# ska-sa/katsdpsigproc

Measured on AMD Instinct MI355X. Metric: visibility samples/s (baselines x channels) through full RFI flagger, higher is better.
Workload: dtype f32 amplitude / f64 deviations

## Files before the change

katsdpsigproc_amd/csrc/fused_common.h:

```cpp
#pragma once
#include <stdlib.h>

#include "bitplane.h"
#include "median_merge.h"
#include "median_window.h"

#ifndef FUSED_MAD_BITS
#define FUSED_MAD_BITS 1
#endif
#ifndef FUSED_STRIP
#define FUSED_STRIP 4
#endif
#define FUSED_THREADS (64 * FUSED_STRIP)
#define FUSED_MAD_NORMAL 1.4826

#ifdef KSP_DIAG_REALTIME
#define FUSED_DIAG_CLOCK() __builtin_amdgcn_s_memrealtime()
#else
#define FUSED_DIAG_CLOCK() __builtin_amdgcn_s_memtime()
#endif
#ifdef KSP_DIAG
#define FUSED_DIAG_STOP(p) ((p).debug_stop)
#define FUSED_DIAG_TRACE(p) ((p).trace)
#else
// ... 621 lines not shown
#pragma unroll
            for (int bit = 6; bit >= 0; bit--) step1(bit);
        } else {
#pragma unroll
            for (int bit = 14; bit >= 0; bit--) step1(bit);
        }
        if (top_hint != nullptr) *top_hint = (int)(K >> 7);
#else
#pragma unroll
        for (int bit = 14; bit >= 2; bit -= 2) step2(bit, bit - 1);
        step1(0);
#endif
        in_bin = ksp_wave_sum_dpp(__popc(eq0) + __popc(eq1));
    } else {
        zeros_keys = zeros;
        if (ksp_any(tiny != 0)) zeros -= ksp_wave_sum(tiny);
        if (zeros == total) return __builtin_nan("");
        rank2 = total + zeros;
        rank = rank2 / 2;
        if (rank < zeros_keys) return 0x1p-150 * FUSED_MAD_NORMAL;
        for (int bit = 14; bit >= 0; bit--) {
            const unsigned test = K | (1u << bit);
            const int c = count_less16<NP>(kp, test);
            if (c <= rank) {
                K = test;
                below_bin = c;
            }
        }
        in_bin = count_less16<NP>(kp, K + 1) - below_bin;
    }
    const bool even = !(rank2 & 1);
    stamp(10);
    if (debug_stop == 32) return (double)(K + below_bin);
    auto key_of = [&](int j) -> unsigned {
        return min((__float_as_uint(dv(j)) & 0x7fffffffu) + 0xffffu, 0x7fffffffu) >> 16;
    };
    auto bin_mask = [&](unsigned key) -> unsigned long long {
        unsigned long long m = 0;
#pragma unroll
        for (int j = 0; j < R; j++)
            if (key_of(j) == key) m |= 1ull << j;
        return m;
    };
    int r = rank - below_bin;
    unsigned long long cand = 0;
    const bool narrowed = in_bin > LIST_CAP;
    if (narrowed) {
        const unsigned first = ((K - 1) << 16) + 1u;
        unsigned offs = 0;
        int below = below_bin;
        for (int bit = 15; bit >= 0; bit--) {
            const unsigned test = first + (offs | (1u << bit));
            int c = 0;
#pragma unroll
            for (int j = 0; j < R; j++) c += (__float_as_uint(dv(j)) & 0x7fffffffu) < test;
            c = ksp_wave_sum(c);
            if (c <= rank) {
                offs |= 1u << bit;
                below = c;
            }
        }
        const unsigned cur = first + offs;
        cand = 0;
#pragma unroll
        for (int j = 0; j < R; j++)
            if ((__float_as_uint(dv(j)) & 0x7fffffffu) == cur) cand |= 1ull << j;
        in_bin = ksp_wave_sum(__popcll(cand));
        r = rank - below;
        below_bin = below;
        if (in_bin > LIST_CAP) {
            auto each = [&](auto &&f) {
                unsigned long long todo = cand;
                while (__any(todo != 0)) {
                    const bool has = todo != 0;
                    const int j = has ? __ffsll((long long)todo) - 1 : 0;
                    todo &= todo - 1;
                    const double x = fabs(exact_dev<WIDTH>(c0 + j, fetch));
                    if (has) f(x);
                }
            };
            double lo = __builtin_inf(), hi = 0.0;
            each([&](double x) {
                lo = fmin(lo, x);
                hi = fmax(hi, x);
            });
            lo = ksp_wave_min(lo);
            hi = ksp_wave_max(hi);
            double xk = lo, prev = lo;
            if (lo != hi) {
                const unsigned long long base = (unsigned long long)__double_as_longlong(lo);
                const unsigned long long span = (unsigned long long)__double_as_longlong(hi) - base;
                unsigned long long offs = 0;
                int below_k = 0;
                for (int bit = 63 - __clzll((long long)span); bit >= 0; bit--) {
                    const unsigned long long test = base + (offs | (1ull << bit));
                    int c = 0;
                    each([&](double x) {
                        c += (unsigned long long)__double_as_longlong(x) < test;
                    });
                    c = ksp_wave_sum(c);
                    if (c <= r) {
                        offs |= 1ull << bit;
                        below_k = c;
                    }
                }
                xk = __longlong_as_double((long long)(base + offs));
                prev = xk;
                if (even && r >= 1 && below_k == r) {
                    double m = 0.0;
                    each([&](double x) { m = (x < xk) ? fmax(m, x) : m; });
                    prev = ksp_wave_max(m);
                }
            }
            if (even && r == 0) {
                float b32 = 0.0f;
#pragma unroll
                for (int j = 0; j < R; j++) {
                    const float a = fabsf(dv(j));
                    b32 = (__float_as_uint(a) < cur) ? fmaxf(b32, a) : b32;
                }
                b32 = ksp_wave_max(b32);
                unsigned long long bm = 0;
#pragma unroll
                for (int j = 0; j < R; j++)
                    if (fabsf(dv(j)) == b32) bm |= 1ull << j;
                const int n2 = gather_exact<WIDTH>(bm, c0, list, 0, LIST_CAP, fetch);
                double below_max = 0.0;
                for (int i = lane; i < min(n2, LIST_CAP); i += 64) below_max = fmax(below_max, list[i]);
                below_max = ksp_wave_max(below_max);
                __builtin_amdgcn_wave_barrier();
                if (n2 > LIST_CAP) {
                    unsigned long long todo = bm;
                    double m = 0.0;
                    while (__any(todo != 0)) {
                        const bool has = todo != 0;
                        const int j = has ? __ffsll((long long)todo) - 1 : 0;
                        todo &= todo - 1;
                        const double x = fabs(exact_dev<WIDTH>(c0 + j, fetch));
                        m = has ? fmax(m, x) : m;
                    }
                    below_max = ksp_wave_max(m);
                }
                prev = below_max;
            }
            if (even) xk = (xk + prev) / 2.0;
            return xk * FUSED_MAD_NORMAL;
        }
    }
    double xk, prev;
    bool have_prev;
    if (!narrowed && in_bin <= 64) {
        int *lc = (int *)list;
        int n = 0;
        auto place = [&](bool hit, int channel) {
            const unsigned long long m = ksp_ballot(hit);
            const int pos = n + __builtin_amdgcn_mbcnt_hi((unsigned)(m >> 32),
                                                         __builtin_amdgcn_mbcnt_lo((unsigned)m, 0));
            if (hit) lc[pos] = channel;
            n += __popcll(m);
        };
        double x;
        bool ranked = false;
        unsigned *lv = (unsigned *)lc + 128;
        static_assert(LIST_CAP * 2 >= 128 + 64 + 8, "candidate values behind the channel numbers");
        if constexpr (R == 64 && HAVE_EXACT) {
            const int mine = __popc(eq0) + __popc(eq1);
            const int incl = ksp_wave_scan_dpp(mine);
            n = __builtin_amdgcn_readlane(incl, 63);
            int pos = incl - mine;
            unsigned h0 = eq0, h1 = eq1;
            while (ksp_any((h0 | h1) != 0)) {
                const bool has = (h0 | h1) != 0;
                int j = 0;
                if (h0) {
                    j = 2 * (__ffs((int)h0) - 1);
                    h0 &= h0 - 1;
                } else if (h1) {
                    j = 2 * (__ffs((int)h1) - 1) + 1;
                    h1 &= h1 - 1;
                }
                const float v = ksp_select_dev<R>(dev, j);
                if (has) {
                    lc[pos] = (c0 + j) | (((exact >> j) & 1) ? (int)0x80000000 : 0);
                    lv[pos] = __float_as_uint(v) & 0x7fffffffu;
                    pos++;
                }
            }
            if (lane < 8) lv[n + lane] = 0xffffffffu;
            __builtin_amdgcn_fence(__ATOMIC_RELEASE, "wavefront");
            __builtin_amdgcn_wave_barrier();
            const int slot = lane < n ? lane : 0;
            const int e0 = lc[slot];
            const unsigned a32 = lv[slot];
            x = (double)__uint_as_float(a32);
            const bool inexact = lane < n && e0 >= 0;
            stamp(11);
            if (debug_stop == 33) return x;
            if (ksp_any(inexact)) {
                const double xe = fabs(exact_dev<WIDTH>(e0 & 0x7fffffff, fetch));
                x = inexact ? xe : x;
            } else {
                unsigned k32, p32;
                rank_list_u32(lv, a32, n, r, lane, k32, p32, have_prev);
                xk = (double)__uint_as_float(k32);
                prev = (double)__uint_as_float(p32);
                ranked = true;
            }
        } else {
            if constexpr (R == 64) {
                const int mine = __popc(eq0) + __popc(eq1);
                const int incl = ksp_wave_scan_dpp(mine);
                n = __builtin_amdgcn_readlane(incl, 63);
                int pos = incl - mine;
                unsigned h0 = eq0, h1 = eq1;
                while (h0 | h1) {
                    if (h0) {
                        lc[pos++] = c0 + 2 * (__ffs((int)h0) - 1);
                        h0 &= h0 - 1;
                    } else {
                        lc[pos++] = c0 + 2 * (__ffs((int)h1) - 1) + 1;
                        h1 &= h1 - 1;
                    }
                }
            } else {
#pragma unroll
                for (int j = 0; j < R; j++) place(key_of(j) == K, c0 + j);
            }
            __builtin_amdgcn_fence(__ATOMIC_RELEASE, "wavefront");
            __builtin_amdgcn_wave_barrier();
            const int c = lc[lane < n ? lane : 0];
            stamp(11);
            if (debug_stop == 33) return (double)c;
            x = fabs(exact_dev<WIDTH>(c, fetch));
        }
        stamp(12);
        if (!ranked) rank_lanes64(x, n, r, lane, xk, prev, have_prev);
        stamp(13);
        __builtin_amdgcn_wave_barrier();
    } else {
        gather_exact<WIDTH>(narrowed ? cand : bin_mask(K), c0, list, 0, LIST_CAP, fetch);
        rank_in_list(list, in_bin, r, lane, xk, prev, have_prev);
        __builtin_amdgcn_wave_barrier();
    }
    if (even && !have_prev) {
        int k2 = -1;
#pragma unroll
        for (int j = 0; j < R; j++) {
            const int kj = (int)key_of(j);
            k2 = (kj < (int)K) ? max(k2, kj) : k2;
        }
        k2 = wave_max_int(k2);
        const bool below_is_tiny = k2 <= 0;
        unsigned long long bm = bin_mask((unsigned)(below_is_tiny ? 0 : k2));
        float b32 = 0.0f;
#pragma unroll
        for (int j = 0; j < R; j++)
            if ((bm >> j) & 1) b32 = fmaxf(b32, fabsf(dv(j)));
        b32 = ksp_wave_max(b32);
        unsigned long long top = 0;
#pragma unroll
        for (int j = 0; j < R; j++)
            if (((bm >> j) & 1) && fabsf(dv(j)) == b32) top |= 1ull << j;
        bool recompute = true;
        if (below_is_tiny) {
            prev = 0x1p-150;
            recompute = false;
        }
        if constexpr (HAVE_EXACT) {
            if (recompute && !ksp_any((top & ~exact) != 0)) {
                prev = (double)b32;
                recompute = false;
            }
        }
        if (recompute) {
            const int n2 = gather_exact<WIDTH>(top, c0, list, 0, LIST_CAP, fetch);
            double below_max = 0.0;
            for (int i = lane; i < min(n2, LIST_CAP); i += 64) below_max = fmax(below_max, list[i]);
            prev = ksp_wave_max(below_max);
            __builtin_amdgcn_wave_barrier();
            if (n2 > LIST_CAP) {
                double m = 0.0;
                while (__any(top != 0)) {
                    const bool has = top != 0;
                    const int j = has ? __ffsll((long long)top) - 1 : 0;
                    top &= top - 1;
                    const double x = fabs(exact_dev<WIDTH>(c0 + j, fetch));
                    m = has ? fmax(m, x) : m;
                }
                prev = ksp_wave_max(m);
            }
        }
    }
    stamp(14);
    if (even) xk = (xk + prev) / 2.0;
    return xk * FUSED_MAD_NORMAL;
}

template <int WIDTH, class Fetch>
__device__ __noinline__ double exact_dev_call(int c, Fetch fetch)
{
    return exact_dev<WIDTH>(c, fetch);
}

template <int WIDTH, class Fetch>
__device__ __forceinline__ unsigned long long threshold_wide(const FusedParams &p,
                                                             const float (&dev)[64],
                                                             unsigned long long fl,
                                                             unsigned long long ge, double t1,
                                                             bool positive, int lane, int C,
                                                             Fetch &&fetch)
{
    const int c0 = lane * 64;
    float nmax = 0.0f;
#pragma unroll
    for (int j = 0; j < 64; j++) nmax = fmaxf(nmax, -dev[j]);
    nmax = ksp_wave_max(nmax);
    float U[64];
    unsigned Nb[16];
#pragma unroll
    for (int j = 0; j < 64; j++) U[j] = dev[j];
#pragma unroll
    for (int q = 0; q < 16; q++) Nb[q] = 0;
    int lvl = -1;
    float umax = 0.0f;
    bool counted = false;
    auto level = [&](auto s_) {
        constexpr int s = decltype(s_)::value;
        ksp_static_for<s>([&](auto r_) {
            constexpr int r = decltype(r_)::value;
            const float e = __shfl_down(U[r], 1, 64);
#pragma unroll
            for (int j = r; j + s < 64; j += s) U[j] += U[j + s];
            U[r + 64 - s] += e;
        });
        if (counted) {
            if constexpr (s >= 4) {
                constexpr int sq = s / 4;
                ksp_static_for<sq>([&](auto r_) {
                    constexpr int r = decltype(r_)::value;
                    const unsigned e = (unsigned)__shfl_down((int)Nb[r], 1, 64);
#pragma unroll
                    for (int q = r; q + sq < 16; q += sq) Nb[q] += Nb[q + sq];
                    Nb[r + 16 - sq] += e;
                });
            } else {
                const unsigned e = (unsigned)__shfl_down((int)Nb[0], 1, 64);
#pragma unroll
                for (int q = 0; q < 16; q++)
                    Nb[q] += __builtin_amdgcn_alignbyte(q + 1 < 16 ? Nb[(q + 1) % 16] : e, Nb[q], s);
            }
        }
    };
#pragma unroll 1
    for (int k = 0; k < p.n_windows; k++) {
        if (positive && !ksp_any((ge & ~fl) != 0)) break;
        const int w = 1 << k;
        const double scale = k == 0 ? p.scales[0] : k == 1 ? p.scales[1] : k == 2 ? p.scales[2]
                           : k == 3 ? p.scales[3] : k == 4 ? p.scales[4] : k == 5 ? p.scales[5]
                           : k == 6 ? p.scales[6] : p.scales[7];
        const float thrf = (float)(t1 * scale);
        const float limf = __fmul_rn(thrf, (float)w);
        const double limit = (double)limf;
        if (positive && lvl >= 0 && umax < thrf) continue;
        if (lvl < 0) {
            counted = ksp_any(fl != 0);
            {
                const unsigned f_lo = (unsigned)fl, f_hi = (unsigned)(fl >> 32);
#pragma unroll
                for (int j = 0; j < 64; j++)
                    U[j] = (((j < 32 ? f_lo : f_hi) >> (j & 31)) & 1u) ? 0.0f : dev[j];
            }
            float m = U[0];
#pragma unroll
            for (int j = 1; j < 64; j++) m = fmaxf(m, U[j]);
            umax = ksp_wave_max(m);
            if (counted) {
#pragma unroll
                for (int q = 0; q < 16; q++)
                    Nb[q] = ((((unsigned)(fl >> (4 * q))) & 0xfu) * 0x00204081u) & 0x01010101u;
            }
            lvl = 0;
            if (positive && umax < thrf) continue;
        }
        while (lvl < k) {
            switch (lvl) {
            case 0: level(std::integral_constant<int, 1>{}); break;
            case 1: level(std::integral_constant<int, 2>{}); break;
            case 2: level(std::integral_constant<int, 4>{}); break;
            case 3: level(std::integral_constant<int, 8>{}); break;
            case 4: level(std::integral_constant<int, 16>{}); break;
            case 5: level(std::integral_constant<int, 32>{}); break;
            default: level(std::integral_constant<int, 64>{}); break;
            }
            lvl++;
        }
        const int nvalid = C - w + 1 - c0;
        const unsigned long long valid = nvalid >= 64 ? ~0ull : nvalid <= 0 ? 0ull : ((1ull << nvalid) - 1);
        unsigned long long hits = 0, unsure = valid;
        if (positive) {
            unsigned h_lo = 0, h_hi = 0, m_lo = 0, m_hi = 0;
            const float c = (float)w * nmax * 0x1p-18f + (float)w * 0x1p-149f;
            if (counted) {
                const unsigned wq = (unsigned)w * 0x01010101u;
                auto one = [&](auto j_, unsigned &h, unsigned &m) {
                    constexpr int j = decltype(j_)::value;
                    const unsigned left = wq - Nb[j / 4];
                    const float rem = (float)((left >> (8 * (j % 4))) & 0xffu);
                    const float T = rem * thrf;
                    const float hi = __builtin_fmaf(T, 1.0f + 0x1p-18f, c);
                    float lo = __builtin_fmaf(T, 1.0f - 0x1p-18f, -c);
                    lo = (rem == 0.0f) ? __builtin_inff() : lo;
                    h = 2 * h + (U[j] > hi);
                    m = 2 * m + (U[j] > lo);
                };
                ksp_static_for<32>([&](auto i_) { one(std::integral_constant<int, 31 - decltype(i_)::value>{}, h_lo, m_lo); });
                ksp_static_for<32>([&](auto i_) { one(std::integral_constant<int, 63 - decltype(i_)::value>{}, h_hi, m_hi); });
            } else {
                const float hi = __builtin_fmaf(limf, 1.0f + 0x1p-18f, c);
                const float lo = __builtin_fmaf(limf, 1.0f - 0x1p-18f, -c);
#pragma unroll
                for (int j = 31; j >= 0; j--) {
                    h_lo = 2 * h_lo + (U[j] > hi);
                    m_lo = 2 * m_lo + (U[j] > lo);
                }
#pragma unroll
                for (int j = 63; j >= 32; j--) {
                    h_hi = 2 * h_hi + (U[j] > hi);
                    m_hi = 2 * m_hi + (U[j] > lo);
                }
            }
            hits = (((unsigned long long)h_hi << 32) | h_lo) & valid;
            unsure = (((unsigned long long)m_hi << 32) | m_lo) & valid & ~hits;
        }
        if (ksp_any(unsure != 0)) {
            const unsigned long long f1 = __shfl_down(fl, 1, 64), f2 = __shfl_down(fl, 2, 64);
            while (ksp_any(unsure != 0)) {
                const bool has = unsure != 0;
                const int j = has ? __ffsll((long long)unsure) - 1 : 0;
                unsure &= unsure - 1;
                double s = 0.0;
                for (int m = 0; m < w; m++) {
                    const int jj = j + m;
                    const unsigned long long fw = jj < 64 ? fl : jj < 128 ? f1 : f2;
                    const bool sub = (fw >> (jj & 63)) & 1;
                    const double x = exact_dev_call<WIDTH>(c0 + jj, fetch);
                    s += sub ? (double)thrf : x;
                }
                if (has && s > limit) hits |= 1ull << j;
            }
            lvl = -1;
        }
        if (!ksp_any(hits != 0)) continue;
        auto suffix_or = [](unsigned long long t) {
            t |= t >> 1; t |= t >> 2; t |= t >> 4; t |= t >> 8; t |= t >> 16; t |= t >> 32;
            return t;
        };
        unsigned long long add = hits;
        for (int s = 1; s < w && s < 64; s <<= 1) add |= add << s;
        unsigned long long h1 = __shfl_up(hits, 1, 64), h2 = __shfl_up(hits, 2, 64);
        if (lane < 1) h1 = 0;
        if (lane < 2) h2 = 0;
        if (w > 64) {
            add |= h1 ? ~0ull : 0ull;
            add |= suffix_or(h2 >> 1);
        } else if (w > 1) {
            add |= suffix_or(h1 >> (65 - w));
        }
        if (ksp_any((add & ~fl) != 0)) {
            fl |= add;
            lvl = -1;
        }
    }
    return fl;
}


template <int R, int WIDTH, int MAXK = 4, class Fetch>
__device__ __forceinline__ unsigned long long threshold_flags(const FusedParams &p,
                                                              const float (&dev)[R], float dmax,
                                                              double noise64, int lane, int C,
                                                              Fetch &&fetch)
{
    static_assert(R <= 64, "flag mask is 64 bits");
    const int c0 = lane * R;
    unsigned long long fl = 0;
    if (p.threshold_kind == KSP_THRESHOLD_SIMPLE) {
        const double thr = p.n_sigma * noise64;
        if (__any((double)dmax * (1.0 + 0x1p-23) > thr)) {
            unsigned long long unsure = 0;
#pragma unroll
            for (int j = 0; j < R; j++) {
                const double d = (double)dev[j];
                const double slack = fabs(d) * 0x1p-23 + 0x1p-149;
                if (d - slack > thr)
                    fl |= 1ull << j;
                else if (d + slack > thr)
                    unsure |= 1ull << j;
            }
            while (__any(unsure != 0)) {
                const bool has = unsure != 0;
                const int j = has ? __ffsll((long long)unsure) - 1 : 0;
                unsure &= unsure - 1;
                const double d = exact_dev<WIDTH>(c0 + j, fetch);
                if (has && d > thr) fl |= 1ull << j;
            }
        }
        return fl;
    }
    const double t1 = p.n_sigma * noise64;
    static_assert(MAXK == 4 || (MAXK == 8 && R == 64), "windows above 8: lanes of 64 channels");
    constexpr int MAXW = 4;
    float thr[MAXW];
    float thr_min = __builtin_inff();
    bool thr_nan = false;
#pragma unroll
    for (int k = 0; k < MAXK; k++) {
        const float t = (float)(t1 * p.scales[k < KSP_MAX_WINDOWS ? k : 0]);
        if (k < MAXW) thr[k < MAXW ? k : 0] = t;
        if (k < p.n_windows) {
            thr_min = fminf(thr_min, t);
            thr_nan |= (t != t);
        }
    }
    const double cand = (double)thr_min * (1.0 - 0x1p-20);
    const bool positive = thr_min > 0.0f;
    const bool any = !positive || ((double)dmax >= cand);
    if (thr_nan || !__any(any)) return 0;

    unsigned long long gt0, ge;
    {
        unsigned g_lo = 0, g_hi = 0, e_lo = 0, e_hi = 0;
        const float t0 = thr[0], tm = thr_min;
#pragma unroll
        for (int j = (R < 32 ? R : 32) - 1; j >= 0; j--)
            asm("v_cmp_ge_f32 vcc, %1, %2\n\tv_addc_co_u32 %0, vcc, %0, %0, vcc"
                : "+v"(e_lo) : "v"(dev[j]), "v"(tm) : "vcc");
#pragma unroll
        for (int j = R - 1; j >= 32; j--)
            asm("v_cmp_ge_f32 vcc, %1, %2\n\tv_addc_co_u32 %0, vcc, %0, %0, vcc"
                : "+v"(e_hi) : "v"(dev[j < R ? j : 0]), "v"(tm) : "vcc");
        if (ksp_any(dmax > t0)) {
#pragma unroll
            for (int j = (R < 32 ? R : 32) - 1; j >= 0; j--)
                asm("v_cmp_gt_f32 vcc, %1, %2\n\tv_addc_co_u32 %0, vcc, %0, %0, vcc"
                    : "+v"(g_lo) : "v"(dev[j]), "v"(t0) : "vcc");
#pragma unroll
            for (int j = R - 1; j >= 32; j--)
                asm("v_cmp_gt_f32 vcc, %1, %2\n\tv_addc_co_u32 %0, vcc, %0, %0, vcc"
                    : "+v"(g_hi) : "v"(dev[j < R ? j : 0]), "v"(t0) : "vcc");
        }
        gt0 = ((unsigned long long)g_hi << 32) | g_lo;
        ge = ((unsigned long long)e_hi << 32) | e_lo;
    }
    const unsigned long long inband =
        (c0 + R <= C) ? (R == 64 ? ~0ull : ((1ull << R) - 1))
                      : (c0 >= C ? 0ull : ((1ull << (C - c0)) - 1));
    if (positive && !__any(((ge & ~gt0) & inband) != 0)) return gt0 & inband;
    if constexpr (MAXK > 4) return threshold_wide<WIDTH>(p, dev, 0ull, ge, t1, positive, lane, C, fetch);

    float d[R];
#pragma unroll
    for (int j = 0; j < R; j++) d[j] = dev[j];
#pragma unroll
    for (int k = 0; k < MAXW; k++) {
        if (k >= p.n_windows) break;
        const int w = 1 << k;
        const float thrf = thr[k];
        const double limit = (double)__fmul_rn(thrf, (float)w);
        if (ksp_any(fl != 0)) {
#pragma unroll
            for (int j = 0; j < R; j++)
                if ((fl >> j) & 1) d[j] = thrf;
        }
        float ext[7];
#pragma unroll
        for (int m = 0; m < 7; m++) ext[m] = __shfl_down(d[m % R], 1 + m / R, 64);
        unsigned nfl = 0;
#pragma unroll
        for (int m = 0; m < 7; m++) {
            const unsigned long long f = __shfl_down(fl, 1 + m / R, 64);
            nfl |= (unsigned)((f >> (m % R)) & 1) << m;
        }
        unsigned long long need = ~0ull;
        if (positive && R == 64) {
            const unsigned long long hot = ge & ~fl;
            const unsigned long long hot_next = __shfl_down(hot, 1, 64);
            unsigned long long reach = hot;
#pragma unroll
            for (int m = 1; m < w; m++) reach |= (hot >> m) | (lane < 63 ? hot_next << (64 - m) : 0ull);
            need = ((unsigned long long)ksp_wave_or_dpp((unsigned)(reach >> 32)) << 32) |
                   ksp_wave_or_dpp((unsigned)reach);
        }
        unsigned long long hits = 0, unsure = 0;
#pragma unroll
        for (int j = 0; j < R; j++) {
            if (!((need >> j) & 1)) continue;
            double s = 0.0, mag = 0.0;
#pragma unroll
            for (int m = 0; m < w; m++) {
                {
                    const int jj = j + m;
                    const float v = (jj < R) ? d[jj % R] : ext[(jj >= R) ? (jj - R) % 7 : 0];
                    const bool sub = (jj < R) ? ((fl >> (jj % 64)) & 1) : ((nfl >> ((jj >= R) ? (jj - R) % 7 : 0)) & 1);
                    s += (double)v;
                    mag += sub ? 0.0 : fabs((double)v);
                }
            }
            const bool valid = (c0 + j + w <= C);
            const double slack = mag * 0x1p-23 + w * 0x1p-149;
            if (valid) {
                if (s - slack > limit)
                    hits |= 1ull << j;
                else if (s + slack > limit)
                    unsure |= 1ull << j;
            }
        }
        while (__any(unsure != 0)) {
            const bool has = unsure != 0;
            const int j = has ? __ffsll((long long)unsure) - 1 : 0;
            unsure &= unsure - 1;
            double s = 0.0;
            for (int m = 0; m < w; m++) {
                const int jj = j + m;
                const bool sub = (jj < R) ? ((fl >> jj) & 1) : ((nfl >> (jj - R)) & 1);
                const double x = exact_dev<WIDTH>(c0 + jj, fetch);
                s += sub ? (double)thrf : x;
            }
            if (has && s > limit) hits |= 1ull << j;
        }
        unsigned pin = 0;
        if (R >= 7) {
            const unsigned long long prev = __shfl_up(hits, 1, 64);
            if (lane > 0) pin = (unsigned)(prev >> (R >= 7 ? R - 7 : 0)) & 0x7fu;
        } else {
#pragma unroll
            for (int back = 1; back * R < 7 + R; back++) {
                const unsigned long long prev = __shfl_up(hits, back, 64);
                const int sh = 7 - back * R;
                if (lane >= back) pin |= (unsigned)(sh >= 0 ? (prev << sh) : (prev >> (-sh))) & 0x7fu;
            }
        }
        unsigned long long own = hits;
        if (w >= 2) { own |= own << 1; pin |= pin << 1; }
        if (w >= 4) { own |= own << 2; pin |= pin << 2; }
        if (w >= 8) { own |= own << 4; pin |= pin << 4; }
        const unsigned long long comb = own | (unsigned long long)(pin >> 7);
        fl |= comb & (R == 64 ? ~0ull : ((1ull << R) - 1));
    }
    return fl;
}

__device__ __forceinline__ void write_flags(const FusedParams &p, unsigned long long fl, int c0,
                                            int bl, int C)
{
    if (bl >= p.baselines) return;
    const uint8_t fv = (uint8_t)p.flag_value;
    while (fl) {
        const int j = __ffsll((long long)fl) - 1;
        fl &= fl - 1;
        const int c = c0 + j;
        if (c < C) p.flags[(size_t)c * p.flags_stride + bl] = fv;
    }
}
```

katsdpsigproc_amd/csrc/ring_kernel.h:

```cpp
#pragma once
#include "fused_dispatch.h"
#include "launch.h"

#ifndef RING_STOP
#define RING_STOP 0
#endif
#define RING_THREADS 512
#define RING_STRIP 8
#define RING_NSLOT 32
#ifndef RING_G
#define RING_G 4
#endif
#ifndef RING_PRIO
#define RING_PRIO 0
#endif
#ifndef RING_STAGGER
#define RING_STAGGER 0
#endif
#define RING_SLOT_BYTES 4096
#define RING_LIST_DOUBLES 256
#define RING_XCD_GROUP 8

struct RingLayout {
    static constexpr size_t RING_BYTES = (size_t)RING_NSLOT * RING_SLOT_BYTES;
    static constexpr size_t LIST_BYTES = sizeof(double) * RING_LIST_DOUBLES * RING_STRIP;
    static constexpr size_t CTRL_BYTES = 64;
    static constexpr size_t LDS_BYTES = RING_BYTES + LIST_BYTES + CTRL_BYTES;
};

#ifdef RING_TRACE
#define RING_TRACE_STRIPS 24
#define RING_TRACE_SLOTS 16
__device__ unsigned long long ring_trace_buf[256 * 8 * RING_TRACE_STRIPS * RING_TRACE_SLOTS];
#endif

#define RING_WORK_LIST 2
#define RING_WORK_DONE 10

__device__ __forceinline__ int ring_strip_of(int x, int t)
{
    return ((t / RING_XCD_GROUP) * 8 + x) * RING_XCD_GROUP + (t % RING_XCD_GROUP);
}

__device__ __forceinline__ int ring_take(unsigned *work, int x, int n_strips, int t0)
{
    for (int k = 0; k < 8; k++) {
        const int xx = (x + k) & 7;
        const int t = t0 + (int)atomicAdd(&work[RING_WORK_LIST + xx], 1u);
        const int s = ring_strip_of(xx, t);
        if (s < n_strips) return s;
    }
    return -1;
}

__device__ __forceinline__ float ring_from_next(float v, float edge, int lane)
{
    const float r = __shfl_down(v, 1, 64);
    return lane == 63 ? edge : r;
}
__device__ __forceinline__ float ring_from_prev(float v, float edge, int lane)
{
    const float r = __shfl_up(v, 1, 64);
    return lane == 0 ? edge : r;
}

template <int WIDTH>
__global__ __launch_bounds__(RING_THREADS) void flagger_ring_kernel(const FusedParams p)
{
    constexpr int R = 64, W = WIDTH, H = WIDTH / 2;
    constexpr int G = RING_G, NSLOT = RING_NSLOT, STEPS = 64, NCHUNK = STEPS / G;
    constexpr int K = NSLOT / G;
    constexpr int PER_CHUNK = G / 2;
    static_assert(W % 2 == 1 && W <= 13 && 2 * H <= G * 3, "merging median only");
    typedef __attribute__((address_space(3))) void lds_void;
    extern __shared__ __attribute__((aligned(16))) char lds[];
    const int tid = threadIdx.x, lane = tid & 63;
    const int wave = __builtin_amdgcn_readfirstlane(tid >> 6);
    const int C = p.channels;
    double *list = (double *)(lds + RingLayout::RING_BYTES) + wave * RING_LIST_DOUBLES;
    int *ctrl = (int *)(lds + RingLayout::RING_BYTES + RingLayout::LIST_BYTES);
    const unsigned lds_base = (unsigned)(size_t)(lds_void *)lds;

    const int q = wave & 3, par = wave >> 2;
    const int rl = lane >> 2;
    const int chunk16 = (lane & 3) ^ ((rl >> 2) & 3);
    const size_t row_bytes = (size_t)p.vis_stride * 8;
    const unsigned lane_off = (unsigned)((size_t)(16 * q + rl) * 64 * row_bytes + (size_t)chunk16 * 16);
    const int pp = wave >> 1, hh = wave & 1;
    const int l16 = lane & 15;
    const unsigned rd_off = (lane >> 4) * 1024 + l16 * 64 + ((pp ^ ((l16 >> 2) & 3)) * 16) + 8 * hh;
    typedef const __attribute__((address_space(3))) char lds_cchar;
    typedef const __attribute__((address_space(3))) unsigned long long lds_cu64;
    lds_cchar *lds3 = (lds_cchar *)(lds_void *)lds;

    unsigned long long run_src = 0;
    const unsigned long long rb2 = 2 * (unsigned long long)row_bytes;
    const unsigned piece_base = __builtin_amdgcn_readfirstlane(lds_base + q * 1024);
    auto issue = [&](int slot) {
        unsigned pb = piece_base;
        asm volatile("" : "+s"(pb));
        const unsigned dst = pb + (unsigned)(slot + par) * RING_SLOT_BYTES;
        unsigned keep;
        asm volatile("s_mov_b32 %0, m0\n\ts_mov_b32 m0, %3\n\ts_nop 0\n\t"
                     "global_load_lds_dwordx4 %1, %2\n\ts_mov_b32 m0, %0"
                     : "=&s"(keep) : "v"(lane_off), "s"(run_src), "s"(dst) : "memory");
        run_src += rb2;
    };
    auto strip_base = [&](int strip) -> const char * {
        return (const char *)p.vis + (size_t)strip * (RING_STRIP * 8);
    };

    const int xcd = blockIdx.x & 7;
    const int per_list = (int)gridDim.x >> 3;
    const int t0 = p.n_static * per_list;
    auto static_strip = [&](int k) { return ring_strip_of(xcd, k * per_list + ((int)blockIdx.x >> 3)); };
    if (tid == 0) {
        int s0 = 0 < p.n_static ? static_strip(0) : ring_take(p.work, xcd, p.n_strips, t0);
        int s1 = -1;
        if (s0 >= 0) s1 = 1 < p.n_static ? static_strip(1) : ring_take(p.work, xcd, p.n_strips, t0);
        ctrl[0] = s0;
        ctrl[1] = s1;
    }
    __syncthreads();
    int cur = __builtin_amdgcn_readfirstlane(ctrl[0]), nxt = __builtin_amdgcn_readfirstlane(ctrl[1]);
    int k_strip = 0;
    auto finish = [&]() {
        if (tid == 0 && atomicAdd(&p.work[RING_WORK_DONE], 1u) == gridDim.x - 1u) {
#pragma unroll
            for (int k = RING_WORK_LIST; k <= RING_WORK_DONE; k++) p.work[k] = 0;
        }
    };
    if (cur < 0) {
        finish();
        return;
    }
#if RING_STAGGER > 0
    if ((blockIdx.x >> 3) & 1) {
#pragma unroll
        for (int i = 0; i < RING_STAGGER; i++) __builtin_amdgcn_s_sleep(127);
    }
#endif
    auto start_of = [&](int strip) -> unsigned long long {
        const unsigned long long a = (unsigned long long)strip_base(strip) + (unsigned long long)par * row_bytes;
        return ((unsigned long long)(unsigned)__builtin_amdgcn_readfirstlane((unsigned)(a >> 32)) << 32) |
               (unsigned long long)(unsigned)__builtin_amdgcn_readfirstlane((unsigned)a);
    };
    run_src = start_of(cur);
#pragma unroll
    for (int j = 0; j < NSLOT; j += 2) issue(j);
    float2 zz[2][G];
    auto read_chunk = [&](int chunk, float2 (&z)[G]) {
        unsigned ro = rd_off + ((chunk * G) % NSLOT) * RING_SLOT_BYTES;
        asm volatile("" : "+v"(ro));
#pragma unroll
        for (int g = 0; g < G; g++) {
            const unsigned long long w = *(lds_cu64 *)(lds3 + ro + g * RING_SLOT_BYTES);
            z[g] = make_float2(__uint_as_float((unsigned)w), __uint_as_float((unsigned)(w >> 32)));
        }
    };
    auto convert_chunk = [&](const float2 (&z)[G], float *a, unsigned &um) {
        static_assert(G == 4, "the pin below names four results");
        unsigned key = ~0u;
#pragma unroll
        for (int g = 0; g < G; g++) key &= ksp_abs_range_key(z[g].x, z[g].y);
#pragma unroll
        for (int g = 0; g < G; g += 2)
            ksp_abs_c64_inrange_x2(z[g].x, z[g].y, z[g + 1].x, z[g + 1].y, a[g], a[g + 1]);
        asm volatile("" : "+v"(a[0]), "+v"(a[1]), "+v"(a[2]), "+v"(a[3]));
        if (ksp_any((key & KSP_ABS_RANGE_BIT) == 0)) {
#pragma unroll
            for (int g = 0; g < G; g++) {
                a[g] = ksp_abs_c64(z[g].x, z[g].y);
                um = max(um, __float_as_uint(a[g]));
            }
        }
    };
    float amp_nxt[G];
    unsigned umax_nxt = 0;
    {
        constexpr int AH0 = (K - 1) * PER_CHUNK;
        __builtin_amdgcn_s_waitcnt(0x0070 | (AH0 & 15) | ((AH0 >> 4) << 14));
        __syncthreads();
        read_chunk(0, zz[0]);
        convert_chunk(zz[0], amp_nxt, umax_nxt);
    }
    const float nanv = __builtin_nanf("");
    const float2 *visf = (const float2 *)p.vis;

#if RING_PRIO == 1
    if (wave >= 4) __builtin_amdgcn_s_setprio(1);
#endif
    int mad_hint = -1;
    const int lane_id = lane;
#ifdef RING_TRACE
    int trace_it = 0;
#define RING_STAMP(i)                                                                              \
    do {                                                                                           \
        if (lane_id == 0 && trace_it < RING_TRACE_STRIPS && blockIdx.x < 256)                      \
            ring_trace_buf[((blockIdx.x * 8 + wave) * RING_TRACE_STRIPS + trace_it) * RING_TRACE_SLOTS + (i)] =   \
                __builtin_amdgcn_s_memtime();                                                      \
    } while (0)
#else
#define RING_STAMP(i) do { } while (0)
#endif
    for (;;) {
        int lane = lane_id;
        asm volatile("" : "+v"(lane));
        const int bl = cur * RING_STRIP + wave;
        const bool more = nxt >= 0;
        const unsigned long long start_nxt = start_of(more ? nxt : cur);
        auto fetch = [&](int c) -> float {
            const bool inside = c >= 0 && c < C;
            const int cc = inside ? c : 0;
            const float2 v = visf[(size_t)cc * p.vis_stride + bl];
            float a = ksp_abs_c64(v.x, v.y);
            return inside ? a : nanv;
        };
        RING_STAMP(0);
#ifdef RING_TRACE
        unsigned long long wait_dma = 0, wait_bar = 0;
        if (lane_id == 0 && trace_it < RING_TRACE_STRIPS && blockIdx.x < 256)
            ring_trace_buf[((blockIdx.x * 8 + wave) * RING_TRACE_STRIPS + trace_it) * RING_TRACE_SLOTS + 4] = __builtin_amdgcn_s_memrealtime();
#endif
        float amp[STEPS];
        unsigned umax = umax_nxt;
        umax_nxt = 0;
#pragma unroll
        for (int g = 0; g < G; g++) amp[g] = amp_nxt[g];
        auto load_chunk = [&](auto more_, auto c_) {
            constexpr bool MORE = decltype(more_)::value;
            constexpr int c = decltype(c_)::value;
            constexpr int AH = (K - 3) * PER_CHUNK;
#ifdef RING_TRACE
            unsigned long long w0;
            asm volatile("s_memtime %0\n\ts_waitcnt lgkmcnt(0)" : "=s"(w0));
#endif
            if constexpr (MORE || (c + K - 1) * G + G <= STEPS)
                __builtin_amdgcn_s_waitcnt(0x0070 | (AH & 15) | ((AH >> 4) << 14));
            else
                __builtin_amdgcn_s_waitcnt(0x0070);
#ifdef RING_TRACE
            unsigned long long w1;
            asm volatile("s_memtime %0\n\ts_waitcnt lgkmcnt(0)" : "=s"(w1));
#endif
#ifndef RING_NOSYNC
            __syncthreads();
#endif
#ifdef RING_TRACE
            unsigned long long w2;
            asm volatile("s_memtime %0\n\ts_waitcnt lgkmcnt(0)" : "=s"(w2));
            wait_dma += w1 - w0;
            wait_bar += w2 - w1;
#endif
            ksp_static_for<G / 2>([&](auto u_) {
                constexpr int j = c * G + 2 * decltype(u_)::value + NSLOT;
                if constexpr (j < STEPS) {
                    issue(j % NSLOT);
                } else if constexpr (MORE) {
                    if constexpr (j == STEPS) run_src = start_nxt;
                    issue(j % NSLOT);
                }
            });
            if constexpr (c == 0) read_chunk(1, zz[1]);
            if constexpr (c + 2 < NCHUNK || (MORE && c + 2 == NCHUNK)) read_chunk(c + 2, zz[c & 1]);
#if RING_PRIO == 2
            if ((c + (wave >> 2)) & 1)
                __builtin_amdgcn_s_setprio(1);
            else
                __builtin_amdgcn_s_setprio(0);
#endif
            if constexpr (c + 1 < NCHUNK)
                convert_chunk(zz[(c + 1) & 1], &amp[(c + 1) * G], umax);
            else if constexpr (MORE)
                convert_chunk(zz[(c + 1) & 1], amp_nxt, umax_nxt);
        };

        float dev[R];
        float dmax;
        unsigned ex_a = 0, ex_b = 0;
        int tiny = 0;
        auto note_exact = [&](unsigned &acc, float x, float m, float d) {
            unsigned t;
            asm("v_min_u32 %1, %2, %3\n\tv_or_b32 %1, 0x7fffff, %1\n\t"
                "v_cmp_ge_f32 vcc, %1, |%4|\n\tv_addc_co_u32 %0, vcc, %0, %0, vcc"
                : "+v"(acc), "=&v"(t)
                : "v"(__float_as_uint(x)), "v"(__float_as_uint(m)), "v"(d)
                : "vcc");
        };
        auto stream = [&](auto more_) __attribute__((always_inline)) {
#if RING_STOP == 1
            dmax = 0.f;
            ksp_static_for<NCHUNK>([&](auto c_) {
                load_chunk(more_, c_);
                constexpr int c = decltype(c_)::value;
#pragma unroll
                for (int g = 0; g < G; g++) {
                    dev[c * G + g] = amp[c * G + g];
                    dmax += amp[c * G + g];
                }
            });
#else
            MergeMedian<R, W> mm;
            mm.pinf = __builtin_inff();
            mm.ninf = -__builtin_inff();
            asm volatile("" : "+v"(mm.pinf), "+v"(mm.ninf));
            const float pinf = mm.pinf, ninf = mm.ninf;
            const bool first = lane == 0, last = lane == 63;
            dmax = ninf;
            float rh[H];
            auto X = [&](auto i_) -> float {
                constexpr int i = decltype(i_)::value;
                if constexpr (i < STEPS) {
                    if constexpr (i % G == 0) load_chunk(more_, std::integral_constant<int, i / G>{});
                    return amp[i];
                } else {
                    if constexpr (i == STEPS) {
#pragma unroll
                        for (int k = 0; k < H; k++)
                            rh[k] = ring_from_next(amp[k], (k & 1) ? ninf : pinf, lane);
                    }
                    return rh[i - STEPS];
                }
            };
            constexpr int RV = R - H;
            constexpr int STAGES = (RV + W - 1) / W;
            using MM = MergeMedian<R, W>;
            float cur_b[W];
            ksp_static_for<W>([&](auto k_) { cur_b[decltype(k_)::value] = X(k_); });
            ksp_static_for<STAGES>([&](auto m_) {
                constexpr int m = decltype(m_)::value;
                float S[MM::S_SIZE];
                S[MM::off(W - 1)] = cur_b[W - 1];
                ksp_static_for<W - 1>([&](auto u_) {
                    constexpr int t = W - 2 - decltype(u_)::value;
                    mm.template insert<W - 1 - t>(&S[MM::off(t + 1)], cur_b[t], &S[MM::off(t)]);
                });
                float P[W], nxt_b[W];
                ksp_static_for<W>([&](auto t_) {
                    constexpr int t = decltype(t_)::value;
                    constexpr int jv = m * W + t;
                    if constexpr (jv < RV) {
                        constexpr int j = jv + H;
                        if constexpr (t >= 1) {
                            nxt_b[t - 1] = X(std::integral_constant<int, (m + 1) * W + t - 1>{});
                            if constexpr (t == 1)
                                P[0] = nxt_b[0];
                            else
                                mm.template insert<t - 1>(P, nxt_b[t - 1], P);
                        }
                        const float med = mm.template rank<W - t, t, H>(&S[MM::off(t)], P);
                        const float xc = (t + H < W) ? cur_b[t + H < W ? t + H : 0] : nxt_b[t + H >= W ? t + H - W : 0];
                        float d = xc - med;
                        constexpr bool right_odd = j + H >= R && ((j + H - R + 1) & 1);
                        if constexpr (right_odd) {
                            const float lo = mm.template rank<W - t, t, H - 1>(&S[MM::off(t)], P);
                            if (last) {
                                const double dd = (double)xc - ((double)lo + (double)med) * 0.5;
                                d = (float)dd;
                                tiny += (d == 0.0f && dd != 0.0);
                            }
                        }
                        asm volatile("" : "+v"(d));
                        if constexpr (jv < 32)
                            note_exact(ex_a, xc, med, d);
                        else
                            note_exact(ex_b, xc, med, d);
                        if constexpr (jv & 1)
                            asm("v_max3_f32 %0, %0, %1, %2" : "+v"(dmax) : "v"(dev[j - 1]), "v"(d));
                        else if constexpr (jv == RV - 1)
                            dmax = mm.vmax(dmax, d);
                        dev[j] = d;
                    }
                });
                if constexpr (m + 1 < STAGES) {
                    ksp_static_for<W>([&](auto k_) {
                        constexpr int k = decltype(k_)::value;
                        constexpr int i = (m + 1) * W + k;
                        constexpr bool have = (m * W + k + 1 < RV) && (k + 1 < W);
                        if constexpr (!have) {
                            if constexpr (i < R + H)
                                nxt_b[k] = X(std::integral_constant<int, i>{});
                            else
                                nxt_b[k] = pinf;
                        }
                    });
#pragma unroll
                    for (int k = 0; k < W; k++) cur_b[k] = nxt_b[k];
                }
            });
            if constexpr (H >= 1) {
                float L[H];
#pragma unroll
                for (int k = 0; k < H; k++)
                    L[k] = ring_from_prev(amp[STEPS - H + k], ((H - k) & 1) ? pinf : ninf, lane);
                constexpr auto soff = [](int j) { return j * H - j * (j - 1) / 2; };
                float SL[H * (H + 1) / 2];
                SL[soff(H - 1)] = L[H - 1];
                ksp_static_for<H - 1>([&](auto u_) {
                    constexpr int j = H - 2 - decltype(u_)::value;
                    mm.template insert<H - 1 - j>(&SL[soff(j + 1)], L[j], &SL[soff(j)]);
                });
                float PL[2 * H];
                PL[0] = amp[0];
                ksp_static_for<H>([&](auto k_) {
                    constexpr int k = decltype(k_)::value + 1;
                    mm.template insert<k>(PL, amp[k], PL);
                });
                ksp_static_for<H>([&](auto j_) {
                    constexpr int j = decltype(j_)::value;
                    if constexpr (j >= 1) mm.template insert<j + H>(PL, amp[j + H], PL);
                    const float med = mm.template rank<H - j, j + H + 1, H>(&SL[soff(j)], PL);
                    const float xc = amp[j];
                    float d = xc - med;
                    if constexpr ((H - j) & 1) {
                        const float lo = mm.template rank<H - j, j + H + 1, H - 1>(&SL[soff(j)], PL);
                        if (first) {
                            const double dd = (double)xc - ((double)lo + (double)med) * 0.5;
                            d = (float)dd;
                            tiny += (d == 0.0f && dd != 0.0);
                        }
                    }
                    note_exact(ex_b, xc, med, d);
                    dmax = mm.vmax(dmax, d);
                    dev[j] = d;
                });
            }
#endif
        };
        if (more)
            stream(std::true_type{});
        else
            stream(std::false_type{});
        RING_STAMP(1);
#ifdef RING_TRACE
        if (lane_id == 0 && trace_it < RING_TRACE_STRIPS && blockIdx.x < 256) {
            ring_trace_buf[((blockIdx.x * 8 + wave) * RING_TRACE_STRIPS + trace_it) * RING_TRACE_SLOTS + 5] = wait_dma;
            ring_trace_buf[((blockIdx.x * 8 + wave) * RING_TRACE_STRIPS + trace_it) * RING_TRACE_SLOTS + 6] = wait_bar;
        }
#endif
        unsigned long long exact;
        {
            const unsigned ra = __builtin_bitreverse32(ex_a), rb = __builtin_bitreverse32(ex_b);
            exact = ((unsigned long long)ra << H) |
                    ((unsigned long long)(rb & ((1u << (32 - H)) - 1u)) << (H + 32)) |
                    (unsigned long long)(rb >> (32 - H));
            unsigned long long first_odd = 0, last_odd = 0;
#pragma unroll
            for (int j = 0; j < H; j++)
                if ((H - j) & 1) first_odd |= 1ull << j;
#pragma unroll
            for (int j = R - H; j < R; j++)
                if ((j + H - R + 1) & 1) last_odd |= 1ull << j;
            if (lane == 0) exact &= ~first_odd;
            if (lane == 63) exact &= ~last_odd;
        }
        if (ksp_any(umax >= 0x7f800000u)) {
            float a2[R + 2 * H];
            int c_first = lane * R - H;
            asm volatile("" : "+v"(c_first));
#pragma unroll
            for (int i = 0; i < R + 2 * H; i++) a2[i] = fetch(c_first + i);
            tiny = 0;
            median_phase_src<R, W>([&](int i) { return a2[i + H]; }, dev, dmax, &tiny);
            exact = 0;
        }
        const bool ticket = more && k_strip + 2 >= p.n_static;
        unsigned t_own = 0;
        if (tid == 0 && ticket) t_own = atomicAdd(&p.work[RING_WORK_LIST + xcd], 1u);

#if RING_STOP == 1 || RING_STOP == 2
        {
            float acc = dmax;
#pragma unroll
            for (int j = 0; j < R; j++) acc += dev[j];
            if (acc == 12345.678f && p.noise != nullptr) p.noise[bl] = acc;
        }
#else
        const double noise64 = mad_noise<R, W, RING_LIST_DOUBLES, true>(dev, lane, list, fetch, RING_STOP > 30 ? RING_STOP : 0,
#ifdef RING_TRACE
                                                                      (trace_it < RING_TRACE_STRIPS && blockIdx.x < 256)
                                                                          ? &ring_trace_buf[((blockIdx.x * 8 + wave) * RING_TRACE_STRIPS + trace_it) * RING_TRACE_SLOTS]
                                                                          : nullptr,
#else
                                                                      nullptr,
#endif
                                                                      exact, &mad_hint, tiny);
        if (lane == 0 && p.noise != nullptr) p.noise[bl] = (float)noise64;
        RING_STAMP(2);
#if RING_STOP == 3 || RING_STOP > 30
        if (noise64 == 12345.678 && p.noise != nullptr) p.noise[bl] = dmax;
#else
        const unsigned long long fl = threshold_flags<R, W>(p, dev, dmax, noise64, lane, C, fetch);
        write_flags(p, fl, lane * R, bl, C);
        RING_STAMP(3);
#endif
#endif

#ifdef RING_TRACE
        if (lane_id == 0 && trace_it < RING_TRACE_STRIPS && blockIdx.x < 256)
            ring_trace_buf[((blockIdx.x * 8 + wave) * RING_TRACE_STRIPS + trace_it) * RING_TRACE_SLOTS + 7] = (unsigned long long)cur + 1;
        trace_it++;
#endif
        if (!more) break;
        cur = nxt;
        if (!ticket) {
            nxt = static_strip(k_strip + 2);
#ifdef RING_END_SYNC
            __syncthreads();
#endif
        } else {
            if (tid == 0) {
                int take = ring_strip_of(xcd, t0 + (int)t_own);
                if (take >= p.n_strips) take = ring_take(p.work, (xcd + 1) & 7, p.n_strips, t0);
                ctrl[2] = take;
            }
            __syncthreads();
            nxt = __builtin_amdgcn_readfirstlane(ctrl[2]);
            __syncthreads();
        }
        k_strip++;
    }
    finish();
}

inline bool ring_supported(const FusedParams &p, int width)
{
    return p.channels == 4096 && width % 2 == 1 && width >= 3 && width <= 13 && !p.is_amplitude &&
           p.flags_mode == KSP_FLAGS_NONE && p.deviations == nullptr && p.work != nullptr &&
           p.baselines >= RING_STRIP && (p.vis_stride % 2) == 0 &&
           (p.threshold_kind != KSP_THRESHOLD_SUM || p.n_windows <= 4) &&
           (size_t)p.vis_stride * 8 * 4096 < 0x7fffff00ull;
}

template <int WIDTH>
inline int launch_ring(int device, hipStream_t s, const FusedParams &p_in, int n_cu, hipEvent_t ev0,
                       hipEvent_t ev1)
{
    FusedParams p = p_in;
    p.n_strips = p.baselines / RING_STRIP;
    auto kern = flagger_ring_kernel<WIDTH>;
    int rc = ksp_lds_opt_in<flagger_ring_kernel<WIDTH>>(device, RingLayout::LDS_BYTES);
    if (rc != 0) return rc;
    const int grid = p.n_strips < n_cu ? p.n_strips : n_cu;
    p.n_static = 0;
    if (grid % 8 == 0 && p.n_strips / grid >= 3) {
        const int by_share = p.n_strips / grid - 2;
        const int by_range = (8 * (p.n_strips / 64)) / (grid / 8);
        p.n_static = by_share < by_range ? by_share : by_range;
    }
#ifndef RING_STATIC
    p.n_static = 0;
#endif
#ifdef RING_TRACE
    {
        void *tb = nullptr;
        KSP_CHECK(hipGetSymbolAddress(&tb, HIP_SYMBOL(ring_trace_buf)));
        KSP_CHECK(hipMemsetAsync(tb, 0, sizeof(ring_trace_buf), s));
    }
#endif
    rc = ksp_launch_timed(kern, dim3(grid), dim3(RING_THREADS), RingLayout::LDS_BYTES, s, ev0, ev1, p);
    if (rc != 0) return rc;
#ifdef RING_TRACE
    if (const char *path = getenv("KSP_RING_TRACE")) {
        KSP_CHECK(hipStreamSynchronize(s));
        const size_t n = sizeof(ring_trace_buf);
        void *host = malloc(n);
        KSP_CHECK(hipMemcpyFromSymbol(host, HIP_SYMBOL(ring_trace_buf), n));
        FILE *f = fopen(path, "wb");
        if (f != nullptr) {
            fwrite(host, 1, n, f);
            fclose(f);
        }
        free(host);
    }
#endif
    return 0;
}
```

Measured before the change: 364.8 billion.

## Route ring kernel wide thresholding through a noinline out-of-line helper

The ring kernel now calls threshold_flags with MAXK=8 and a RingWide policy. When no channel exceeds the first threshold, or when more than four windows are configured, thresholding goes to a separate __noinline__ function that takes the deviations and window scales by value. Otherwise the existing inline 4-window path still runs. The fetch lambda becomes a plain struct so it can be passed to that function. The aim is to keep the large threshold_wide code out of the hot kernel body and lower register pressure, at the cost of call overhead and copying 64 floats plus the scales on each out-of-line call.

```diff
diff --git a/katsdpsigproc_amd/csrc/fused_common.h b/katsdpsigproc_amd/csrc/fused_common.h
--- a/katsdpsigproc_amd/csrc/fused_common.h
+++ b/katsdpsigproc_amd/csrc/fused_common.h
@@ -947,8 +947,8 @@
     return exact_dev<WIDTH>(c, fetch);
 }
 
-template <int WIDTH, class Fetch>
-__device__ __forceinline__ unsigned long long threshold_wide(const FusedParams &p,
+template <int WIDTH, class Params, class Fetch>
+__device__ __forceinline__ unsigned long long threshold_wide(const Params &p,
                                                              const float (&dev)[64],
                                                              unsigned long long fl,
                                                              unsigned long long ge, double t1,
@@ -1120,7 +1120,7 @@
 }
 
 
-template <int R, int WIDTH, int MAXK = 4, class Fetch>
+template <int R, int WIDTH, int MAXK = 4, class WIDE = void, class Fetch>
 __device__ __forceinline__ unsigned long long threshold_flags(const FusedParams &p,
                                                               const float (&dev)[R], float dmax,
                                                               double noise64, int lane, int C,
@@ -1201,7 +1201,12 @@
         (c0 + R <= C) ? (R == 64 ? ~0ull : ((1ull << R) - 1))
                       : (c0 >= C ? 0ull : ((1ull << (C - c0)) - 1));
     if (positive && !__any(((ge & ~gt0) & inband) != 0)) return gt0 & inband;
-    if constexpr (MAXK > 4) return threshold_wide<WIDTH>(p, dev, 0ull, ge, t1, positive, lane, C, fetch);
+    if constexpr (MAXK > 4) {
+        if constexpr (std::is_void<WIDE>::value)
+            return threshold_wide<WIDTH>(p, dev, 0ull, ge, t1, positive, lane, C, fetch);
+        else if (!ksp_any(gt0 != 0) || p.n_windows > 4)
+            return WIDE::template run<WIDTH>(p, dev, ge, t1, positive, lane, C, fetch);
+    }
 
     float d[R];
 #pragma unroll
diff --git a/katsdpsigproc_amd/csrc/ring_kernel.h b/katsdpsigproc_amd/csrc/ring_kernel.h
--- a/katsdpsigproc_amd/csrc/ring_kernel.h
+++ b/katsdpsigproc_amd/csrc/ring_kernel.h
@@ -63,6 +63,52 @@
     const float r = __shfl_up(v, 1, 64);
     return lane == 0 ? edge : r;
 }
+
+struct RingFetch {
+    const float2 *vis;
+    int stride, bl, channels;
+    __device__ __forceinline__ float operator()(int c) const
+    {
+        const bool inside = c >= 0 && c < channels;
+        const int cc = inside ? c : 0;
+        const float2 v = vis[(size_t)cc * stride + bl];
+        const float a = ksp_abs_c64(v.x, v.y);
+        return inside ? a : __builtin_nanf("");
+    }
+};
+
+struct RingDeviations {
+    float v[64];
+};
+struct RingWindows {
+    int n_windows;
+    double scales[KSP_MAX_WINDOWS];
+};
+template <int WIDTH>
+__device__ __noinline__ unsigned long long ring_threshold_wide(RingDeviations d, RingWindows w,
+                                                               unsigned long long ge, double t1,
+                                                               bool positive, int lane, int C,
+                                                               RingFetch fetch)
+{
+    return threshold_wide<WIDTH>(w, d.v, 0ull, ge, t1, positive, lane, C, fetch);
+}
+struct RingWide {
+    template <int WIDTH>
+    __device__ static __forceinline__ unsigned long long run(const FusedParams &p, const float (&dev)[64],
+                                                             unsigned long long ge, double t1,
+                                                             bool positive, int lane, int C,
+                                                             const RingFetch &fetch)
+    {
+        RingDeviations d;
+#pragma unroll
+        for (int j = 0; j < 64; j++) d.v[j] = dev[j];
+        RingWindows w;
+        w.n_windows = p.n_windows;
+#pragma unroll
+        for (int k = 0; k < KSP_MAX_WINDOWS; k++) w.scales[k] = p.scales[k];
+        return ring_threshold_wide<WIDTH>(d, w, ge, t1, positive, lane, C, fetch);
+    }
+};
 
 template <int WIDTH>
 __global__ __launch_bounds__(RING_THREADS) void flagger_ring_kernel(const FusedParams p)
@@ -184,7 +230,6 @@
         read_chunk(0, zz[0]);
         convert_chunk(zz[0], amp_nxt, umax_nxt);
     }
-    const float nanv = __builtin_nanf("");
     const float2 *visf = (const float2 *)p.vis;
 
 #if RING_PRIO == 1
@@ -209,13 +254,7 @@
         const int bl = cur * RING_STRIP + wave;
         const bool more = nxt >= 0;
         const unsigned long long start_nxt = start_of(more ? nxt : cur);
-        auto fetch = [&](int c) -> float {
-            const bool inside = c >= 0 && c < C;
-            const int cc = inside ? c : 0;
-            const float2 v = visf[(size_t)cc * p.vis_stride + bl];
-            float a = ksp_abs_c64(v.x, v.y);
-            return inside ? a : nanv;
-        };
+        const RingFetch fetch = {visf, p.vis_stride, bl, C};
         RING_STAMP(0);
 #ifdef RING_TRACE
         unsigned long long wait_dma = 0, wait_bar = 0;
@@ -490,7 +529,7 @@
 #if RING_STOP == 3 || RING_STOP > 30
         if (noise64 == 12345.678 && p.noise != nullptr) p.noise[bl] = dmax;
 #else
-        const unsigned long long fl = threshold_flags<R, W>(p, dev, dmax, noise64, lane, C, fetch);
+        const unsigned long long fl = threshold_flags<R, W, 8, RingWide>(p, dev, dmax, noise64, lane, C, fetch);
         write_flags(p, fl, lane * R, bl, C);
         RING_STAMP(3);
 #endif
```

Result: no change. 366.9 billion, median of 6 (+0.6%).
